# tlemane/kmtricks

Measured on AMD Instinct MI355X. Metric: k-mers merged/s (merge stage, sum over partitions of input records / time), higher is better.
Workload: dtype u64 keys / u32 counts (integer)

## Files before the change

kmtricks_amd/csrc/kmx_api.hip:

```cpp
#include "kmx_host.hpp"

#include <algorithm>
#include <chrono>
#include <cmath>
#include <sys/mman.h>
#include <unordered_map>
#include <mutex>
#include <cstdlib>
#include <cstring>
#include <memory>

using namespace kmx;

static thread_local std::string g_create_err;

void* kmx_ctx::dalloc(size_t bytes)
{
  if (bytes == 0) bytes = 256;
  if (bytes >= (8u << 20)) { size_t p2 = (size_t)1 << 23; while (p2 * 2 <= bytes) p2 *= 2; const size_t q = p2 >> 3; bytes = (bytes + q - 1) / q * q; }
  int best = -1;
  for (size_t i = 0; i < pool.size(); i++)
    if (!pool[i].used && pool[i].bytes >= bytes && pool[i].bytes <= 2 * bytes + (1u << 20) &&
        (best < 0 || pool[i].bytes < pool[best].bytes)) best = (int)i;
  if (best >= 0) { pool[best].used = true; return pool[best].p; }
// ... 388 lines not shown
  size_t o_recs = 0, o_len = 0, o_smin = 0, o_bounds = 0, o_stats = 0, o_ctrl = 0, o_segs = 0;
  u8* d_out = nullptr; size_t out_bytes = 0;
  u16* d_rowrec = nullptr;
  u32 bft_c = 1;
  u8* d_img = nullptr; size_t img_bytes = 0;
  u64 t_rows = 0, t_cols = 0;
  Seg* d_segs = nullptr;
  Seg* d_segs_own = nullptr;
  u64 rows = 0, nsegs = 0;
  bool done = false;
  bool handed_back = false;
  u32 nblk = 0, nb = 0, rt_cols = 0, slots_cap = 0;
  size_t o_skel = 0, o_nskel = 0, o_rbounds = 0;
  u8* d_ov = nullptr;
  size_t o_spdir = 0;
  size_t o_ovx = 0; u32 xcap = 0;
  u64 sparse_rows = 0;
  u8* d_body = nullptr;
  bool body_ready = false;
  hipEvent_t ev_body = nullptr;
  void* d_body_tmp = nullptr;
  u8* d_dense = nullptr; u32 dpitch = 0, dense_cap = 0; size_t o_gbase = 0;
  u8* d_narrow = nullptr; u32 npitch = 0;
  u64 row_keys = 0;
  bool ordered = false;
  std::vector<u32> src;
  int kernel = 0;
};

struct kmx_merge_result {
// ... 94 lines not shown
    const TaskDev* d_subs = reinterpret_cast<const TaskDev*>(R->d_meta + R->o_subtasks);
    const uint2* d_subitems = reinterpret_cast<const uint2*>(R->d_meta + R->o_subitems);
    const ColsDev* d_cols = reinterpret_cast<const ColsDev*>(R->d_meta + R->o_cols);
    const uint2* d_citems = reinterpret_cast<const uint2*>(R->d_meta + R->o_citems);
    static const bool overlap = getenv("KMX_COLS_PREP_OVERLAP") != nullptr;
    hipStream_t ps = overlap ? ctx->aux : ctx->stream;
    if (!R->ev_pre) KMX_HIP(ctx, hipEventCreateWithFlags(&R->ev_pre, hipEventDisableTiming));
    if (overlap && ctx->stream_shared) {
      KMX_HIP(ctx, hipEventRecord(R->ev_pre, ctx->stream));
      KMX_HIP(ctx, hipStreamWaitEvent(ctx->aux, R->ev_pre, 0));
    }
    if (!overlap) KMX_HIP(ctx, hipStreamWaitEvent(ctx->stream, R->ev_up, 0));
    KMX_HIP(ctx, launch_range_bounds(kw, d_subs, nt, R->sub_max_n, R->sub_max_c, ps));
    KMX_HIP(ctx, CO.skel(d_subs, d_subitems, R->n_subitems, ps));
    KMX_HIP(ctx, CO.prep(d_tasks, d_subs, d_cols, nt, ps));
    KMX_HIP(ctx, hipEventRecord(R->ev_pre, ps));
    KMX_HIP(ctx, hipStreamWaitEvent(ctx->stream, R->ev_up, 0));
    KMX_HIP(ctx, launch_range_bounds(kw, d_tasks, nt, R->max_n, R->max_c, ctx->stream));
    KMX_HIP(ctx, hipStreamWaitEvent(ctx->stream, R->ev_pre, 0));
    if (R->ev0) KMX_HIP(ctx, hipEventRecord(R->ev0, ctx->stream));
    const u32 cols_grid_env = getenv("KMX_COLS_GRID") ? (u32)atoi(getenv("KMX_COLS_GRID")) : 0u;
    const u32 sparse_cus_env = getenv("KMX_SPARSE_CUS") ? (u32)atoi(getenv("KMX_SPARSE_CUS")) : 0u;
    KMX_HIP(ctx, CO.merge(mode, (R->cols_ext ? 1 : 0) | (R->cols_resc ? 2 : 0) | (R->cols_ord ? 4 : 0) | (R->cols_narrow ? 8 : 0), d_tasks, d_cols, d_citems, R->n_citems, d_ticket,
                          cols_grid_env ? std::min(cols_grid_env, R->cols_grid) : R->cols_grid, ctx->stream));
    if (R->ev0) { if (!R->ev_mid) KMX_HIP(ctx, hipEventCreate(&R->ev_mid)); KMX_HIP(ctx, hipEventRecord(R->ev_mid, ctx->stream)); }
    KMX_HIP(ctx, CO.sparse(mode | (R->cols_resc ? 2 : 0) | (R->cols_ord ? 4 : 0), d_tasks, d_cols, d_items, R->n_items, nt, d_ticket, sparse_cus_env ? std::min(sparse_cus_env, (u32)ctx->n_cu) : (u32)ctx->n_cu, ctx->stream));
    if (R->share_fix) {
      if ((size_t)R->max_n * 4 > 48 * 1024) KMX_HIP(ctx, hipFuncSetAttribute(reinterpret_cast<const void*>(&k_share_fix), hipFuncAttributeMaxDynamicSharedMemorySize, (int)std::min<size_t>((size_t)R->max_n * 4, 160 * 1024)));
      hipLaunchKernelGGL(k_share_fix, dim3((unsigned)ctx->n_cu * 2u, nt), dim3(256), (size_t)R->max_n * 4, ctx->stream, (const TaskDev*)d_tasks, kw);
      KMX_HIP(ctx, hipGetLastError());
// ... 357 lines not shown
  R->d_meta = (u8*)ctx->dalloc(off);
  R->h_meta = (u8*)ctx->halloc(upload_bytes);
  if (!R->d_meta || !R->h_meta) { ctx->dfree(R->d_meta); ctx->hfree(R->h_meta); return ctx->fail(KMX_E_NOMEM, "meta allocation failed"); }
  auto drop_blocks = [&]() {
    for (auto& G : R->tasks) { ctx->dfree(G.d_out); ctx->dfree(G.d_ov); ctx->dfree(G.d_img); ctx->dfree(G.d_rowrec); ctx->dfree(G.d_dense); ctx->dfree(G.d_narrow); }
    for (auto& G : R->subs) ctx->dfree(G.d_out);
    ctx->dfree(R->d_meta); ctx->hfree(R->h_meta); ctx->dfree(R->d_rem); R->d_rem = nullptr;
  };
  bool narrow_failed = false;
  for (auto& H : R->tasks) {
    H.d_out = (u8*)ctx->dalloc(H.out_bytes);
    if (H.d_out && cols) {
      H.xcap = (u32)std::min<u64>(0x7FFFFF00ULL, CO.ext_entries(H.slots_cap, H.nblk));
      H.o_ovx = align_up((size_t)(CO.scratch_keys(H.slots_cap, H.nblk) * 8 + CO.scratch_counts(H.slots_cap, H.nblk) * 8), 256);
      H.o_spdir = align_up(H.o_ovx + (size_t)H.xcap * (CO.key_words + 1) * 8, 256);
      H.d_ov = (u8*)ctx->dalloc(H.o_spdir + 256 + (size_t)CO.dir_bytes(H.slots_cap));
      if (H.d_ov && hipMemsetAsync(H.d_ov + H.o_spdir, 0, 256 + (size_t)CO.dir_bytes(H.slots_cap), ctx->aux) != hipSuccess) { ctx->dfree(H.d_ov); H.d_ov = nullptr; }
      if (R->cols_ord) {
        const TaskHost& Q = R->subs[&H - R->tasks.data()];
        u64 longest = 0, sum = 0; for (u32 l : Q.len) { longest = std::max<u64>(longest, l); sum += l; }
        u64 cap = (H.rec_min <= 1 ? std::min<u64>(sum, longest * 5 / 2) : longest * 3 / 2) + 4096;
        if (ctx->keys_per_longest > 0.0) cap = std::max<u64>(cap, (u64)(ctx->keys_per_longest * 1.25 * (double)longest) + 4096);
        H.dense_cap = (u32)std::min<u64>(std::min<u64>(cap, H.out_cap_rows), 0xFFFFFF00ULL);
        H.dpitch = (u32)align_up(H.row_bytes - 8 * kw, 8);
        H.d_dense = (u8*)ctx->dalloc((size_t)H.dense_cap * H.dpitch);
        if (R->cols_narrow) {
          H.npitch = (u32)align_up((size_t)H.N, 16) + 16;
          H.d_narrow = (u8*)ctx->dalloc((size_t)H.dense_cap * H.npitch);
          if (!H.d_narrow) narrow_failed = true;
        }
      }
// ... 61 lines not shown
      }
      fill_dev(Q, sd[t]);
      sd[t].item0 = si;
      for (u32 j = 0; j < Q.c; j++) sitems[si++] = make_uint2(t, j);
      ColsDev& C = cd[t];
      C.skel = reinterpret_cast<u64*>(R->d_meta + H.o_skel);
      C.nskel = reinterpret_cast<u32*>(R->d_meta + H.o_nskel);
      C.rbounds = reinterpret_cast<u32*>(R->d_meta + H.o_rbounds);
      C.ovkeys = reinterpret_cast<u64*>(H.d_ov);
      C.ovcnt = reinterpret_cast<u32*>(H.d_ov + CO.scratch_keys(H.slots_cap, H.nblk) * 8);
      C.ovx = reinterpret_cast<u64*>(H.d_ov + H.o_ovx);
      C.xcur = reinterpret_cast<u32*>(H.d_ov + H.o_spdir);
      C.xcap = H.xcap;
      C.spdir = H.d_ov + H.o_spdir + 256;
      C.slots_cap = H.slots_cap; C.nblk = H.nblk; C.nb = H.nb; C.rt = H.rt_cols;
      if (R->cols_ord) {
        const size_t ng = CO.groups(H.slots_cap);
        C.dense = H.d_dense; C.dpitch = H.dpitch; C.dense_cap = H.dense_cap;
        C.dnarrow = H.d_narrow; C.npitch = H.npitch;
        C.gbase = reinterpret_cast<u32*>(R->d_meta + H.o_gbase);
        C.chain = reinterpret_cast<u64*>(H.d_ov + H.o_spdir + 256);
        C.gmap = reinterpret_cast<uint4*>(H.d_ov + H.o_spdir + 256 + ng * 8);
        C.gmax = reinterpret_cast<u32*>(R->d_meta + R->o_ticket) + 2;
        C.ngcap = (u32)ng;
        u32* const tk3 = reinterpret_cast<u32*>(R->h_meta + R->o_ticket) + 3;
        *tk3 = std::max<u32>(*tk3, (u32)ng);
      }
      for (u32 j = 0; j < H.c * H.nblk; j++) citems[ci++] = make_uint2(t, j);
    }
  }
// ... 450 lines not shown
    st[5 * (u64)N + i] = two + twr;
  }
  return KMX_OK;
}

#ifdef KMX_PHASE_PROF
namespace kmx { void rows_phase_prof_dump(); void pivot_phase_prof_dump(); void bft_phase_prof_dump(); }
#endif
extern "C" void kmx_result_free(kmx_merge_result* R)
{
  if (!R) return;
  kmx_ctx* ctx = R->ctx;
  (void)hipSetDevice(ctx->device);
  if (R->ev_done) (void)hipEventSynchronize(R->ev_done);
  else (void)hipStreamSynchronize(ctx->stream);
#ifdef KMX_PHASE_PROF
  const ColsOps& CO = cols_ops((int)R->tasks[0].kw);
  if (R->is_bft) kmx::bft_phase_prof_dump();
  if (!R->is_bf) { if (R->use_cols) { if (CO.phase_prof_dump) CO.phase_prof_dump(); } else if (R->use_pivot) kmx::pivot_phase_prof_dump(); else kmx::rows_phase_prof_dump(); }
#endif
  for (auto& H : R->tasks) {
    if (H.ev_body) { (void)hipEventSynchronize(H.ev_body); (void)hipEventDestroy(H.ev_body); }
    ctx->dfree(H.d_out); ctx->dfree(H.d_segs_own); ctx->dfree(H.d_ov); ctx->dfree(H.d_img); ctx->dfree(H.d_rowrec); ctx->dfree(H.d_body); ctx->dfree(H.d_body_tmp); ctx->dfree(H.d_dense); ctx->dfree(H.d_narrow);
  }
  for (auto& Q : R->subs) ctx->dfree(Q.d_out);
  ctx->dfree(R->d_meta);
  ctx->hfree(R->h_meta);
  ctx->dfree(R->d_in);
  ctx->dfree(R->d_rem);
  if (R->ev_in) (void)hipEventDestroy(R->ev_in);
// ... 548 lines not shown
```

kmtricks_amd/csrc/kmx_dev.hpp:

```cpp
#pragma once
#include <hip/hip_runtime.h>
#include <stdint.h>

namespace kmx {

typedef unsigned long long u64;
typedef uint32_t u32;
typedef uint16_t u16;
typedef uint8_t u8;
typedef __attribute__((address_space(1))) const u32 gu32;

struct Seg {
  u32 range;
  u32 seq;
  u64 row_off;
  u32 nrows;
  u32 pad;
};

struct TaskDev {
  const u8* const* recs;
  const u32* len;
  const u32* soft_min;
  u32* bounds;
// ... 28 lines not shown
  void* spdir;
  u32 slots_cap;
  u32 nblk;
  u32 nb;
  u32 rt;
  u8* dense;
  u32 dpitch;
  u32 dense_cap;
  u8* dnarrow;
  u32 npitch;
  u32* gbase;
  u64* chain;
  uint4* gmap;
  u32* gmax;
  u32 ngcap;
};

#ifndef KMX_CHUNK_BYTES
#define KMX_CHUNK_BYTES 262144
#endif

enum { ERR_ROWS_OVERFLOW = 1, ERR_SEGS_OVERFLOW = 2, ERR_FALLBACK = 4,
       ERR_DIVERGENT = 8,
       ERR_SLICES = 16,
       ERR_DENSE_CAP = 32 };

template <int KW> struct Key { u64 w[KW]; };

template <int KW> __device__ __forceinline__ bool key_less(const Key<KW>& a, const Key<KW>& b) {
#pragma unroll
// ... 67 lines not shown
```

kmtricks_amd/csrc/kmx_host.hpp:

```cpp
#pragma once
#include <hip/hip_runtime.h>
#include <string>
#include <functional>
#include <vector>
#include "kmx_dev.hpp"
#include "skf.hpp"
#include "../../include/kmx.h"

namespace kmx {

int rows_lds_bytes(int kw, u32 n_lists);
int rows_cap(int kw, u32 n_lists);
int rows_wgs_per_cu(int kw);
u32 rows_chunk_rows(u32 row_bytes);
u32 rows_image_bytes(int kw);
hipError_t launch_range_bounds(int kw, const TaskDev* tasks, u32 n_tasks, u32 max_n, u32 max_c, hipStream_t st);
hipError_t launch_merge_rows(int kw, int mode, const TaskDev* tasks, const uint2* items, u32 n_items, u32* ticket,
                             u32 grid_x, u32 max_n, hipStream_t st);
int rows_s_cap(int kw, u32 n_lists);
int rows_s_wgs_per_cu(int kw);
u32 rows_s_image_bytes(int kw);
hipError_t launch_merge_rows_s(int kw, int mode, const TaskDev* tasks, const uint2* items, u32 n_items, u32* ticket, u32 grid_x, u32 max_n, hipStream_t st);
int pivot_lds_bytes(int kw);
u32 pivot_max_lists();
hipError_t launch_merge_pivot(int kw, int mode, const TaskDev* tasks, const uint2* items, u32 n_items, u32* ticket,
                              u32 grid_x, hipStream_t st);
struct ColsOps {
  int (*lds_bytes)();
  u32 (*block_lists)();
  u32 (*wgs_per_cu)();
  u32 (*tile_rows)(u32 nb);
  u64 (*scratch_keys)(u32 slots, u32 nblk);
  u64 (*scratch_counts)(u32 slots, u32 nblk);
  u64 (*ext_entries)(u32 slots, u32 nblk);
  u32 (*skel_cap)();
  hipError_t (*skel)(const TaskDev* subs, const uint2* items, u32 n_items, hipStream_t st);
  hipError_t (*prep)(const TaskDev* tasks, const TaskDev* subs, const ColsDev* cols, u32 n_tasks, hipStream_t st);
  hipError_t (*merge)(int mode, int ext, const TaskDev* tasks, const ColsDev* cols, const uint2* items, u32 n_items, u32* ticket, u32 grid_x, hipStream_t st);
  hipError_t (*sparse)(int mode, const TaskDev* tasks, const ColsDev* cols, const uint2* range_items, u32 n_items, u32 n_tasks, u32* ticket, u32 n_cu, hipStream_t st);
  u64 (*dir_bytes)(u32 slots);
  u32 (*groups)(u32 slots);
  hipError_t (*offsets)(const ColsDev* cols, u32 task, u64* goff, hipStream_t st);
  hipError_t (*gather)(const TaskDev* tasks, const ColsDev* cols, u32 task, u32 n_groups, const u64* goff, u8* body, hipStream_t st);
  hipError_t (*order)(const TaskDev* tasks, const ColsDev* cols, u32 task, u32 n_groups, const u64* goff, u32* order, hipStream_t st);
  void (*dbg_dump)();
  void (*phase_prof_dump)();
  u32 key_words;
};
const ColsOps& cols_ops_k1();
const ColsOps& cols_ops_k2();
inline const ColsOps& cols_ops(int kw) { return kw == 2 ? cols_ops_k2() : cols_ops_k1(); }
int bf_lds_bytes(u32 rt, u32 nb, u32 n_lists);
hipError_t launch_range_bounds_bf(const TaskDev* tasks, u32 n_tasks, u32 max_n, u32 max_c, hipStream_t st);
hipError_t launch_merge_bf(int bfc, const TaskDev* tasks, const uint2* items, u32 n_items, u32* ticket,
                           u32 grid_x, int lds, hipStream_t st);
u32 bft_tile_rows(u32 rec_min, u32 share_min);
u32 bft_block_lists();
u32 bft_max_lists();
u32 bft_round_records(bool wide);
u32 bft_fit_rows(u32 max_n, bool bits);
// ... 182 lines not shown
```

kmtricks_amd/csrc/merge_cols.hip:

```cpp
#include "kmx_host.hpp"
#include <algorithm>
#include <cstdio>
#include <cstring>

#ifndef KMX_CL_KW
#define KMX_CL_KW 1
#endif
#if KMX_CL_KW == 1
#define CLNS cols_k1
#elif KMX_CL_KW == 2
#define CLNS cols_k2
#elif KMX_CL_KW == 3
#define CLNS cols_k3
#else
#define CLNS cols_k4
#endif

namespace kmx { namespace CLNS {

#ifndef KMX_CL_TPB
#define KMX_CL_TPB 1024
#endif
constexpr int CL_TPB = KMX_CL_TPB;
constexpr int CL_WGS = 1024 / CL_TPB;
// ... 3 lines not shown
constexpr int CL_G = KMX_CL_G;
constexpr int KW = KMX_CL_KW;
constexpr int RB = KW * 8 + 4;
constexpr int RD = RB / 4;
constexpr int EW = KW + 1;
constexpr int CL_U = KW == 1 ? 16 : 8;
constexpr int CL_W = CL_G * CL_U;
constexpr int CL_NB = CL_TPB / CL_G;
constexpr int CL_IMG = 61440 / CL_WGS;
constexpr int CL_RT = CL_W * 7 / 8;
constexpr int CL_KPL = (CL_RT + 63) / 64;
constexpr int CL_NT = (CL_KPL == 1 && CL_WGS == 1 && KW == 1) ? 2 : 1;
constexpr int CL_PT = CL_KPL == 1 ? 2048 : 4096;
constexpr int CL_PTSHIFT = CL_PT == 2048 ? 21 : 20;
constexpr int CL_HALVES = CL_KPL;
constexpr int CL_SEEDS = 256;
constexpr int CL_OVW = 128;
constexpr int CL_XS = 3 * CL_OVW;
constexpr int CL_NW = CL_TPB / 64;
constexpr int CK_BITS = 1 << 17;
constexpr int CP_MAXSEG = 2048;

__device__ u32 kmx_cols_dbg[16];

namespace {

typedef u32 u32x3 __attribute__((ext_vector_type(3), aligned(4)));
typedef u32 u32x4 __attribute__((ext_vector_type(4), aligned(4)));
typedef __attribute__((address_space(1))) const u32x3 gu32x3;
typedef __attribute__((address_space(1))) const u32x4 gu32x4;
typedef __attribute__((address_space(1))) u64 gu64w;
// ... 60 lines not shown
  return ((u32)__umul24(x, hf) >> CL_PTSHIFT) & (u32)(CL_PT - 1);
}
__device__ __forceinline__ u32 cl_mult(u32 seed)
{
  if (KW == 2 && seed >= 16u) return 0x80000000u | (seed - 15u);
  if (seed >= 64u) return 0x80000000u | (seed - 63u);
  return ((0x9E3779u + seed * 0x5A6B2u) & 0xFFFFFFu) | ((13u + (seed * 7u) % 19u) << 24);
}
__device__ __forceinline__ u32 cl_mix(CKey key)
{
  const u64 k = ck_fold(key);
  u32 x = (u32)k ^ ((u32)(k >> 32) * 0x9E3779B1u);
  x *= 0x85EBCA6Bu; x ^= x >> 15; x *= 0x2C1B3C6Du; x ^= x >> 13;
  return x;
}
__device__ __forceinline__ u32 cl_build(ClEnt* tab, const CKey (&key)[CL_KPL], const bool (&have)[CL_KPL], u32 lane, u32 (&slot)[CL_KPL])
{
  for (u32 s = 0; s < (u32)CL_SEEDS; s++) {
    const u32 mult = cl_mult(s);
    u32 h[CL_KPL], old[CL_KPL];
    bool clash = false;
#pragma unroll
    for (int x = 0; x < CL_KPL; x++) {
      h[x] = cl_thash(key[x], mult);
      old[x] = have[x] ? atomicCAS(&tab[h[x]].idx, 0u, lane + 64u * x + 1) : 0u;
      clash |= old[x] != 0;
    }
    if (__ballot(clash) == 0) {
#pragma unroll
      for (int x = 0; x < CL_KPL; x++) { if (have[x]) ent_set(tab[h[x]], key[x]); slot[x] = h[x]; }
      return mult;
    }
#pragma unroll
    for (int x = 0; x < CL_KPL; x++) if (have[x] && old[x] == 0) atomicExch(&tab[h[x]].idx, 0u);
  }
  return 0;
}

}

#ifndef KMX_SK_TPB
#define KMX_SK_TPB 256
#endif
constexpr int SK_TPB = KMX_SK_TPB;
constexpr int SK_CAP = 2048;

__global__ __launch_bounds__(SK_TPB)
void k_cols_skel(const TaskDev* __restrict__ subs, const uint2* __restrict__ items, u32 n_items)
{
  __shared__ CKey ks[SK_CAP];
  __shared__ u32 wsum[SK_TPB / 64];
// ... 156 lines not shown
      u32 g = 0;
      for (u32 j = 0; j < T.c; j++) { C.gbase[j] = g; const u32 n = C.rbounds[j + 1] - C.rbounds[j]; g += max(1u, (n + C.rt - 1) / C.rt) * (u32)CL_HALVES; }
      C.gbase[T.c] = g; s_ng = g;
      atomicMax(C.gmax, g);
    }
    __syncthreads();
    const u32 ng = s_ng;
    for (u32 g = tid; g < ng; g += CP_TPB) {
      u32 lo = 0, hi = T.c;
      while (hi - lo > 1) { const u32 mid = (lo + hi) >> 1; if (C.gbase[mid] <= g) lo = mid; else hi = mid; }
      C.gmap[g] = make_uint4(lo + 1, g - C.gbase[lo], C.rbounds[lo], C.rbounds[lo + 1]);
    }
  }
}

__device__ const u32 kmx_cols_sentinel[8] = {~0u, ~0u, KW == 1 ? 0u : ~0u, KW == 1 ? 0u : ~0u, 0u, 0u, 0u, 0u};

#ifdef KMX_PHASE_PROF
__device__ u64 kmx_cols_prof[8];
__device__ u64 kmx_sparse_prof[8];
#ifndef KMX_PROF_TID
#define KMX_PROF_TID 512
#endif
#endif

constexpr u64 CL_NONSOLID = 1ULL << 63;
template <int MODE, bool EXT, bool RESC, bool ORD, bool NAR>
__global__ __launch_bounds__(CL_TPB, CL_WGS)
void k_merge_cols(const TaskDev* __restrict__ tasks, const ColsDev* __restrict__ cols, const uint2* __restrict__ items,
                  u32 n_items, u32* ticket)
{
// ... 54 lines not shown
    const u32 end = on ? T.bounds[(u64)(range + 1) * N + li] : 0u;
    const u32 smin = T.soft_min[li];
    gu32* const base = (gu32*)(uintptr_t)T.recs[li];
    gu32* const sentinel = (gu32*)(uintptr_t)kmx_cols_sentinel;
    CRec rec[CL_U];
#pragma unroll
    for (int u = 0; u < CL_U; u++) {
      const u32 ix = cur + ((r + CL_G * u - cur) & (CL_W - 1));
      rec[u] = cl_none();
      if (ix < end) rec[u] = cl_load(base + (u64)ix * RD);
    }
    u64 tsum = 0; u32 tn = 0;
    u64 rsum = 0; u32 rn = 0;
    const bool rescue = RESC && cl_uni(T.share_min) != 0;
    CKey skn[CL_KPL];
    u32 myslot[CL_KPL];
    bool failed = false;
#pragma unroll
    for (int x = 0; x < CL_KPL; x++) { skn[x] = ck_inf(); myslot[x] = 0; }
    if (tid < 64) {
      bool have[CL_KPL];
#pragma unroll
      for (int x = 0; x < CL_KPL; x++) {
        const u32 j = (u32)tid + 64u * x;
        have[x] = j < rt && s_lo + j < s_hi;
        if (have[x]) {
          skn[x] = skel[s_lo + j];
          if (blk == 0 && !ord) ck_store(reinterpret_cast<u32*>(T.out + (u64)(s_lo + j) * row_bytes), skn[x]);
        }
      }
      const u32 mult = cl_build(ptab, skn, have, (u32)tid, myslot);
      if (tid == 0) { sh[4] = mult; if (mult == 0) { failed = true; atomicAdd(&kmx_cols_dbg[0], 1u); } }
    }
    CKey khi_n = ntiles > 1 ? skel[s_lo + rt] : ck_inf();
    CKey kmid_n = (CL_HALVES > 1 && s_lo + 56 < s_hi) ? skel[s_lo + 56] : ck_inf();
    u32 rnd = 0;
    cl_barrier();
    CLPH(0);

    for (u32 q = 0; q < ntiles; q++) {
      const u32 s0 = s_lo + q * rt;
      const u32 rte = min(rt, s_hi - s0);
      const bool last = cl_uni(q + 1 == ntiles ? 1u : 0u) != 0;
      const CKey khi = ck_uni(khi_n);
      const CKey kmid = ck_uni(kmid_n);
      if (!last) {
        if (tid < 64) {
#pragma unroll
          for (int x = 0; x < CL_KPL; x++) { const u32 j = (u32)tid + 64u * x; skn[x] = ck_inf(); if (j < rt && s0 + rt + j < s_hi) skn[x] = skel[s0 + rt + j]; }
        }
        khi_n = q + 2 < ntiles ? skel[s0 + 2 * rt] : ck_inf();
        kmid_n = (CL_HALVES > 1 && s0 + rt + 56 < s_hi) ? skel[s0 + rt + 56] : ck_inf();
      }
      const ClEnt* const tab = ptab + (q % CL_NT) * CL_PT;
      const u32 mult = cl_uni(sh[4 + (q % CL_NT)]);
      gu64w* const ovk0 = (gu64w*)(uintptr_t)(C.ovkeys + (((((u64)(slot0 + q) * CL_HALVES) * nblk + blk) * CL_NW + wave) * CL_OVW) * EW);
      gu64w* const ovk1 = ovk0 + (u64)nblk * CL_NW * CL_OVW * EW;
      const u64 li_hi = (u64)li << 32;
      u32 wov = 0, wov1 = 0;
      u32 xb0 = 0, xb1 = 0;
      auto extend = [&](u32& xb) {
        u32 b = 0;
        if (lane == 0) b = atomicAdd(C.xcur, (u32)CL_XS);
        b = cl_uni(b);
        xb = (b + (u32)CL_XS <= C.xcap) ? b + 1u : 0xFFFFFFFFu;
      };
      gu64w* const ovx = (gu64w*)(uintptr_t)C.ovx;

      for (;;) {
        if (tid == 0) sh[1 + (rnd == 2 ? 0 : rnd + 1)] = 0;
// ... 107 lines not shown
        const u32 more = cl_uni(sh[1 + rnd]);
        rnd = rnd == 2 ? 0 : rnd + 1;
        if (!more) break;
      }
      if (lane == 0) {
        const u64 s0i = (((u64)(slot0 + q) * CL_HALVES) * nblk + blk) * CL_NW + wave, s1i = (((u64)(slot0 + q) * CL_HALVES + 1) * nblk + blk) * CL_NW + wave;
        reinterpret_cast<uint2*>(C.ovcnt)[s0i] = make_uint2(wov, xb0 == 0xFFFFFFFFu ? 0u : xb0);
        if (CL_HALVES > 1) reinterpret_cast<uint2*>(C.ovcnt)[s1i] = make_uint2(wov1, xb1 == 0xFFFFFFFFu ? 0u : xb1);
        const bool over0 = wov > (u32)CL_OVW && (xb0 - 1u >= 0xFFFFFFFEu || wov > (u32)(CL_OVW + CL_XS));
        const bool over1 = wov1 > (u32)CL_OVW && (xb1 - 1u >= 0xFFFFFFFEu || wov1 > (u32)(CL_OVW + CL_XS));
        if (over0 || over1) {
          if (lane == 0) atomicOr(&T.ctrl[2], (u64)ERR_SLICES); failed = true; atomicAdd(&kmx_cols_dbg[1], 1u); atomicMax(&kmx_cols_dbg[5], max(wov, wov1)); if (last) atomicAdd(&kmx_cols_dbg[6], 1u); if (q == 0) atomicAdd(&kmx_cols_dbg[7], 1u); }
      }

      if (wave == 0) {
        ClEnt* const old = ptab + (q % CL_NT) * CL_PT;
#pragma unroll
        for (int x = 0; x < CL_KPL; x++) if ((u32)lane + 64u * x < rte) old[myslot[x]].idx = 0;
        if (!last) {
          const u32 sn = s0 + rt;
          bool have[CL_KPL];
#pragma unroll
          for (int x = 0; x < CL_KPL; x++) {
            const u32 j = (u32)lane + 64u * x;
            have[x] = j < rt && sn + j < s_hi;
            if (have[x] && blk == 0 && !ord) ck_store(reinterpret_cast<u32*>(T.out + (u64)(sn + j) * row_bytes), skn[x]);
          }
          const u32 m2 = cl_build(ptab + ((q + 1) % CL_NT) * CL_PT, skn, have, (u32)lane, myslot);
          if (lane == 0) { sh[4 + ((q + 1) % CL_NT)] = m2; if (m2 == 0) { failed = true; atomicAdd(&kmx_cols_dbg[0], 1u); } }
        }
      } else {
        if (NAR) {
          const u32 lr = (u32)lane >> 3, lc = (u32)lane & 7u, nch = (nbl + 15u) >> 4;
          for (u32 j = (wave - 1) * 8u + lr; j < rte; j += (CL_NW - 1) * 8u) {
            u8* const nrow = nar + (u64)(s0 + j) * npitch;
            if (lc < nch) {
              uint4* const src = reinterpret_cast<uint4*>(img8 + j * nbs + 16u * lc);
              const uint4 v = *src; *src = make_uint4(0, 0, 0, 0);
              *reinterpret_cast<uint4*>(nrow + col0 + 16u * lc) = v;
            }
            if (lc == 0) { const u8 f = rowbig[j]; rowbig[j] = 0; nrow[npitch - 16u + blk] = f; }
          }
        } else
        if (MODE == 0) {
// ... 55 lines not shown
      }
      if (RESC) {
        u32 rlo = (u32)rsum, rhi = (u32)(rsum >> 32);
        u64 rs = rsum;
#pragma unroll
        for (int off = 1; off < CL_G; off <<= 1) {
          const u32 olo = __shfl_xor(rlo, off), ohi = __shfl_xor(rhi, off);
          rs += (u64)olo | ((u64)ohi << 32);
          rlo = (u32)rs; rhi = (u32)(rs >> 32);
          rn += __shfl_xor(rn, off);
        }
        if (on && r == 0 && rn) { atomicAdd(&T.stats[1 * (u64)N + li], (u64)rn); atomicAdd(&T.stats[5 * (u64)N + li], rs); }
      }
    }
    if (failed) atomicOr(&T.ctrl[2], (u64)ERR_FALLBACK);
    __syncthreads();
  }
}

#ifndef KMX_CK_TPB0
#define KMX_CK_TPB0 256
#endif
#ifndef KMX_CK_TPB1
#define KMX_CK_TPB1 512
#endif
#ifndef KMX_CK_Z
#define KMX_CK_Z 16
#endif
#ifndef KMX_CK_OCC1
#define KMX_CK_OCC1 4
// ... 887 lines not shown
      }
    } else if ((row_bytes & 3u) == 0) for (u32 t = lane; t < row_bytes / 4; t += 64) reinterpret_cast<u32*>(d)[t] = reinterpret_cast<const u32*>(s)[t];
    else for (u32 t = lane; t < row_bytes; t += 64) d[t] = s[t];
  }
}

void cols_dbg_dump()
{
  u32 h[16];
  if (hipMemcpyFromSymbol(h, HIP_SYMBOL(kmx_cols_dbg), sizeof(h)) != hipSuccess) return;
  if (h[9]) fprintf(stderr, "[kmx merge] k_cols_sparse: the group count of the batch was beyond every task's room (%u workgroups stopped at the room)\n", h[9]);
  if (h[8]) fprintf(stderr, "[kmx merge] k_cols_sparse: %u look-backs given up (last: group %u, %u entries still unpublished in front of it)\n", h[8], h[10], h[11]);
  fprintf(stderr, "[kmx merge] k_merge_cols hand-back reasons: no collision-free row table %u, slice overflow %u (wave-tiles; largest %u, in a range's last tile %u, first tile %u), kept key outside the row keys %u, check table full %u, lists too divergent %u (tasks)\n", h[0], h[1], h[5], h[6], h[7], h[2], h[3], h[4]);
  memset(h, 0, sizeof(h)); (void)hipMemcpyToSymbol(HIP_SYMBOL(kmx_cols_dbg), h, sizeof(h));
}
#ifdef KMX_PHASE_PROF
void cols_phase_prof_dump()
{
  u64 h[8];
  if (hipMemcpyFromSymbol(h, HIP_SYMBOL(kmx_cols_prof), sizeof(h)) != hipSuccess) return;
  u64 tot = 0; for (int i = 0; i < 8; i++) tot += h[i];
  static const char* nm[8] = {"item setup", "window wait", "scan", "bar(scan)", "tile out", "bar(out)", "-", "-"};
  for (int i = 0; i < 6; i++) fprintf(stderr, "[cols] %-12s %6.2f%%  %llu\n", nm[i], tot ? 100.0 * h[i] / tot : 0.0, h[i]);
  memset(h, 0, sizeof(h));
  (void)hipMemcpyToSymbol(HIP_SYMBOL(kmx_cols_prof), h, sizeof(h));
  if (hipMemcpyFromSymbol(h, HIP_SYMBOL(kmx_sparse_prof), sizeof(h)) != hipSuccess) return;
  tot = 0; for (int i = 0; i < 8; i++) tot += h[i];
  static const char* sn[8] = {"group entries", "zero maps", "mark twice | sample + place", "candidates | rank", "sort", "runs + claim", "rows", "gather (rec-min 1)"};
  for (int i = 0; i < 8; i++) fprintf(stderr, "[sparse] %-14s %6.2f%%  %llu\n", sn[i], tot ? 100.0 * h[i] / tot : 0.0, h[i]);
  memset(h, 0, sizeof(h));
// ... 9 lines not shown
u64 cols_scratch_keys(u32 slots, u32 nblk) { return (u64)slots * CL_HALVES * nblk * CL_NW * CL_OVW * EW; }
u64 cols_scratch_counts(u32 slots, u32 nblk) { return (u64)slots * CL_HALVES * nblk * CL_NW; }
u64 cols_ext_entries(u32 slots, u32 nblk) { return std::max<u64>(64 * 1024, (u64)slots * CL_HALVES * nblk * CL_NW * CL_OVW / 16); }

u32 cols_skel_cap() { return SK_CAP; }
hipError_t launch_cols_skel(const TaskDev* subs, const uint2* items, u32 n_items, hipStream_t st)
{
  hipLaunchKernelGGL(k_cols_skel, dim3(n_items), dim3(SK_TPB), 0, st, subs, items, n_items);
  return hipGetLastError();
}
hipError_t launch_cols_prep(const TaskDev* tasks, const TaskDev* subs, const ColsDev* cols, u32 n_tasks, hipStream_t st)
{
  hipLaunchKernelGGL(k_cols_prep, dim3(n_tasks), dim3(CP_TPB), 0, st, tasks, subs, cols);
  return hipGetLastError();
}
template <int MODE, bool EXT, bool RESC, bool ORD, bool NAR>
static hipError_t launch_merge_cols_as(const TaskDev* tasks, const ColsDev* cols, const uint2* items, u32 n_items, u32* ticket, u32 grid_x, hipStream_t st)
{
  const int lds = cols_lds_bytes();
  hipError_t e = hipFuncSetAttribute(reinterpret_cast<const void*>(&k_merge_cols<MODE, EXT, RESC, ORD, NAR>), hipFuncAttributeMaxDynamicSharedMemorySize, lds);
  if (e != hipSuccess) return e;
  hipLaunchKernelGGL((k_merge_cols<MODE, EXT, RESC, ORD, NAR>), dim3(grid_x), dim3(CL_TPB), lds, st, tasks, cols, items, n_items, ticket);
  return hipGetLastError();
}
hipError_t launch_merge_cols(int mode, int ext, const TaskDev* tasks, const ColsDev* cols, const uint2* items, u32 n_items, u32* ticket, u32 grid_x, hipStream_t st)
{
  const bool x = ext & 1, r = (ext & 2) != 0, o = (ext & 4) != 0, n = (ext & 8) != 0 && o && mode == 0;
#define KMX_CL_L3(M, X, R) (o ? launch_merge_cols_as<M, X, R, true, false>(tasks, cols, items, n_items, ticket, grid_x, st) : launch_merge_cols_as<M, X, R, false, false>(tasks, cols, items, n_items, ticket, grid_x, st))
#define KMX_CL_LAUNCH(M) (r ? (x ? KMX_CL_L3(M, true, true) : KMX_CL_L3(M, false, true)) : (x ? KMX_CL_L3(M, true, false) : KMX_CL_L3(M, false, false)))
  if (n) return r ? (x ? launch_merge_cols_as<0, true, true, true, true>(tasks, cols, items, n_items, ticket, grid_x, st) : launch_merge_cols_as<0, false, true, true, true>(tasks, cols, items, n_items, ticket, grid_x, st))
// ... 40 lines not shown
  hipLaunchKernelGGL(k_cols_offsets, dim3(1), dim3(1024), 0, st, cols, task, goff);
  return hipGetLastError();
}
hipError_t launch_cols_gather(const TaskDev* tasks, const ColsDev* cols, u32 task, u32 n_groups, const u64* goff, u8* body, hipStream_t st)
{
  hipLaunchKernelGGL(k_cols_gather<true>, dim3(n_groups), dim3(GA_TPB), 0, st, tasks, cols, task, goff, body);
  return hipGetLastError();
}
hipError_t launch_cols_order(const TaskDev* tasks, const ColsDev* cols, u32 task, u32 n_groups, const u64* goff, u32* order, hipStream_t st)
{
  hipLaunchKernelGGL(k_cols_gather<false>, dim3(n_groups), dim3(GA_TPB), 0, st, tasks, cols, task, goff, reinterpret_cast<u8*>(order));
  return hipGetLastError();
}

static const ColsOps g_ops = {cols_lds_bytes, cols_block_lists, cols_wgs_per_cu, cols_tile_rows, cols_scratch_keys, cols_scratch_counts, cols_ext_entries, cols_skel_cap,
                              launch_cols_skel, launch_cols_prep, launch_merge_cols, launch_cols_sparse, cols_dir_bytes, cols_groups, launch_cols_offsets,
                              launch_cols_gather, launch_cols_order, cols_dbg_dump,
#ifdef KMX_PHASE_PROF
                              cols_phase_prof_dump,
#else
                              nullptr,
#endif
                              (u32)KMX_CL_KW};
}
#if KMX_CL_KW == 1
const ColsOps& cols_ops_k1() { return cols_k1::g_ops; }
#elif KMX_CL_KW == 2
const ColsOps& cols_ops_k2() { return cols_k2::g_ops; }
#elif KMX_CL_KW == 3
const ColsOps& cols_ops_k3() { return cols_k3::g_ops; }
#else
const ColsOps& cols_ops_k4() { return cols_k4::g_ops; }
// ... 3 lines not shown
```

Measured before the change: 127.8 billion.

## Precompute collision-free hash seeds per tile in a separate prep kernel

Adds a k_cols_seeds kernel on the prep stream that searches each tile's hash multiplier with an LDS bitmap instead of CAS on the row table, storing seeds in a new per-slot tseed array. The merge kernel then just reads the seed and fills the table directly, dropping the CAS/retry build and per-tile slot clearing in favor of a full table clear at the end. Seed search moves off the critical merge path and can overlap with other prep work, but it adds a kernel launch and extra memory, and raises the try limit to 1024.

```diff
diff --git a/kmtricks_amd/csrc/kmx_api.hip b/kmtricks_amd/csrc/kmx_api.hip
--- a/kmtricks_amd/csrc/kmx_api.hip
+++ b/kmtricks_amd/csrc/kmx_api.hip
@@ -426,6 +426,7 @@
   size_t o_skel = 0, o_nskel = 0, o_rbounds = 0;
   u8* d_ov = nullptr;
   size_t o_spdir = 0;
+  size_t o_tseed = 0;
   size_t o_ovx = 0; u32 xcap = 0;
   u64 sparse_rows = 0;
   u8* d_body = nullptr;
@@ -550,6 +551,12 @@
     KMX_HIP(ctx, launch_range_bounds(kw, d_subs, nt, R->sub_max_n, R->sub_max_c, ps));
     KMX_HIP(ctx, CO.skel(d_subs, d_subitems, R->n_subitems, ps));
     KMX_HIP(ctx, CO.prep(d_tasks, d_subs, d_cols, nt, ps));
+    {
+      u32 max_slots = 0;
+      for (auto& H : R->tasks) max_slots = std::max(max_slots, H.slots_cap);
+      const char* const tenv = getenv("KMX_COLS_SEED_TRIES");
+      KMX_HIP(ctx, CO.seeds(d_tasks, d_cols, nt, max_slots, tenv && atoi(tenv) > 0 ? (u32)atoi(tenv) : 0u, getenv("KMX_TRACE") != nullptr, ps));
+    }
     KMX_HIP(ctx, hipEventRecord(R->ev_pre, ps));
     KMX_HIP(ctx, hipStreamWaitEvent(ctx->stream, R->ev_up, 0));
     KMX_HIP(ctx, launch_range_bounds(kw, d_tasks, nt, R->max_n, R->max_c, ctx->stream));
@@ -937,7 +944,8 @@
       H.xcap = (u32)std::min<u64>(0x7FFFFF00ULL, CO.ext_entries(H.slots_cap, H.nblk));
       H.o_ovx = align_up((size_t)(CO.scratch_keys(H.slots_cap, H.nblk) * 8 + CO.scratch_counts(H.slots_cap, H.nblk) * 8), 256);
       H.o_spdir = align_up(H.o_ovx + (size_t)H.xcap * (CO.key_words + 1) * 8, 256);
-      H.d_ov = (u8*)ctx->dalloc(H.o_spdir + 256 + (size_t)CO.dir_bytes(H.slots_cap));
+      H.o_tseed = align_up(H.o_spdir + 256 + (size_t)CO.dir_bytes(H.slots_cap), 256);
+      H.d_ov = (u8*)ctx->dalloc(H.o_tseed + (size_t)H.slots_cap * 4);
       if (H.d_ov && hipMemsetAsync(H.d_ov + H.o_spdir, 0, 256 + (size_t)CO.dir_bytes(H.slots_cap), ctx->aux) != hipSuccess) { ctx->dfree(H.d_ov); H.d_ov = nullptr; }
       if (R->cols_ord) {
         const TaskHost& Q = R->subs[&H - R->tasks.data()];
@@ -1029,6 +1037,7 @@
       C.xcap = H.xcap;
       C.spdir = H.d_ov + H.o_spdir + 256;
       C.slots_cap = H.slots_cap; C.nblk = H.nblk; C.nb = H.nb; C.rt = H.rt_cols;
+      C.tseed = reinterpret_cast<u32*>(H.d_ov + H.o_tseed);
       if (R->cols_ord) {
         const size_t ng = CO.groups(H.slots_cap);
         C.dense = H.d_dense; C.dpitch = H.dpitch; C.dense_cap = H.dense_cap;
@@ -1509,6 +1518,7 @@
   (void)hipSetDevice(ctx->device);
   if (R->ev_done) (void)hipEventSynchronize(R->ev_done);
   else (void)hipStreamSynchronize(ctx->stream);
+  if (R->use_cols && getenv("KMX_TRACE")) cols_ops((int)R->tasks[0].kw).seeds_dump();
 #ifdef KMX_PHASE_PROF
   const ColsOps& CO = cols_ops((int)R->tasks[0].kw);
   if (R->is_bft) kmx::bft_phase_prof_dump();
diff --git a/kmtricks_amd/csrc/kmx_dev.hpp b/kmtricks_amd/csrc/kmx_dev.hpp
--- a/kmtricks_amd/csrc/kmx_dev.hpp
+++ b/kmtricks_amd/csrc/kmx_dev.hpp
@@ -66,6 +66,7 @@
   uint4* gmap;
   u32* gmax;
   u32 ngcap;
+  u32* tseed;
 };
 
 #ifndef KMX_CHUNK_BYTES
diff --git a/kmtricks_amd/csrc/kmx_host.hpp b/kmtricks_amd/csrc/kmx_host.hpp
--- a/kmtricks_amd/csrc/kmx_host.hpp
+++ b/kmtricks_amd/csrc/kmx_host.hpp
@@ -36,6 +36,7 @@
   u32 (*skel_cap)();
   hipError_t (*skel)(const TaskDev* subs, const uint2* items, u32 n_items, hipStream_t st);
   hipError_t (*prep)(const TaskDev* tasks, const TaskDev* subs, const ColsDev* cols, u32 n_tasks, hipStream_t st);
+  hipError_t (*seeds)(const TaskDev* tasks, const ColsDev* cols, u32 n_tasks, u32 max_slots, u32 max_tries, bool trace, hipStream_t st);
   hipError_t (*merge)(int mode, int ext, const TaskDev* tasks, const ColsDev* cols, const uint2* items, u32 n_items, u32* ticket, u32 grid_x, hipStream_t st);
   hipError_t (*sparse)(int mode, const TaskDev* tasks, const ColsDev* cols, const uint2* range_items, u32 n_items, u32 n_tasks, u32* ticket, u32 n_cu, hipStream_t st);
   u64 (*dir_bytes)(u32 slots);
@@ -44,6 +45,7 @@
   hipError_t (*gather)(const TaskDev* tasks, const ColsDev* cols, u32 task, u32 n_groups, const u64* goff, u8* body, hipStream_t st);
   hipError_t (*order)(const TaskDev* tasks, const ColsDev* cols, u32 task, u32 n_groups, const u64* goff, u32* order, hipStream_t st);
   void (*dbg_dump)();
+  void (*seeds_dump)();
   void (*phase_prof_dump)();
   u32 key_words;
 };
diff --git a/kmtricks_amd/csrc/merge_cols.hip b/kmtricks_amd/csrc/merge_cols.hip
--- a/kmtricks_amd/csrc/merge_cols.hip
+++ b/kmtricks_amd/csrc/merge_cols.hip
@@ -41,7 +41,6 @@
 constexpr int CL_PT = CL_KPL == 1 ? 2048 : 4096;
 constexpr int CL_PTSHIFT = CL_PT == 2048 ? 21 : 20;
 constexpr int CL_HALVES = CL_KPL;
-constexpr int CL_SEEDS = 256;
 constexpr int CL_OVW = 128;
 constexpr int CL_XS = 3 * CL_OVW;
 constexpr int CL_NW = CL_TPB / 64;
@@ -132,27 +131,33 @@
   x *= 0x85EBCA6Bu; x ^= x >> 15; x *= 0x2C1B3C6Du; x ^= x >> 13;
   return x;
 }
-__device__ __forceinline__ u32 cl_build(ClEnt* tab, const CKey (&key)[CL_KPL], const bool (&have)[CL_KPL], u32 lane, u32 (&slot)[CL_KPL])
-{
-  for (u32 s = 0; s < (u32)CL_SEEDS; s++) {
+__device__ __forceinline__ u32 cl_find(u32* bm, const CKey (&key)[CL_KPL], const bool (&have)[CL_KPL], u32 lane, u32 max_tries, u32& tries)
+{
+  for (u32 s = 0; s < max_tries; s++) {
     const u32 mult = cl_mult(s);
-    u32 h[CL_KPL], old[CL_KPL];
+    for (u32 w = lane; w < (u32)CL_PT / 32u; w += 64u) bm[w] = 0;
+    __builtin_amdgcn_wave_barrier();
     bool clash = false;
 #pragma unroll
     for (int x = 0; x < CL_KPL; x++) {
-      h[x] = cl_thash(key[x], mult);
-      old[x] = have[x] ? atomicCAS(&tab[h[x]].idx, 0u, lane + 64u * x + 1) : 0u;
-      clash |= old[x] != 0;
-    }
-    if (__ballot(clash) == 0) {
-#pragma unroll
-      for (int x = 0; x < CL_KPL; x++) { if (have[x]) ent_set(tab[h[x]], key[x]); slot[x] = h[x]; }
-      return mult;
-    }
-#pragma unroll
-    for (int x = 0; x < CL_KPL; x++) if (have[x] && old[x] == 0) atomicExch(&tab[h[x]].idx, 0u);
-  }
+      const u32 h = cl_thash(key[x], mult);
+      if (have[x]) clash |= ((atomicOr(&bm[h >> 5], 1u << (h & 31u)) >> (h & 31u)) & 1u) != 0;
+    }
+    __builtin_amdgcn_wave_barrier();
+    if (__ballot(clash) == 0) { tries = s + 1; return mult; }
+  }
+  tries = max_tries;
   return 0;
+}
+__device__ __forceinline__ void cl_fill(ClEnt* tab, const CKey (&key)[CL_KPL], const bool (&have)[CL_KPL], u32 lane, u32 mult)
+{
+#pragma unroll
+  for (int x = 0; x < CL_KPL; x++) {
+    if (have[x]) {
+      ClEnt e; memset(&e, 0, sizeof(e)); ent_set(e, key[x]); e.idx = lane + 64u * x + 1;
+      tab[cl_thash(key[x], mult)] = e;
+    }
+  }
 }
 
 }
@@ -339,7 +344,52 @@
   }
 }
 
-__device__ const u32 kmx_cols_sentinel[8] = {~0u, ~0u, KW == 1 ? 0u : ~0u, KW == 1 ? 0u : ~0u, 0u, 0u, 0u, 0u};
+constexpr int CS_TPB = 256;
+constexpr u32 CS_TRIES = 1024;
+__device__ u32 kmx_cols_tries[12];
+__global__ __launch_bounds__(CS_TPB)
+void k_cols_seeds(const TaskDev* __restrict__ tasks, const ColsDev* __restrict__ cols, u32 max_tries, u32 trace)
+{
+  __shared__ u32 bm[CS_TPB / 64][CL_PT / 32];
+  __shared__ u32 s_fail;
+  const TaskDev& T = tasks[blockIdx.y];
+  const ColsDev& C = cols[blockIdx.y];
+  const u32 tid = threadIdx.x, lane = tid & 63u, wave = tid >> 6;
+  if (tid == 0) s_fail = 0;
+  if (__syncthreads_or((__hip_atomic_load(&T.ctrl[2], __ATOMIC_RELAXED, __HIP_MEMORY_SCOPE_AGENT) & (u64)(ERR_FALLBACK | ERR_ROWS_OVERFLOW)) != 0)) return;
+  const u32 slot = blockIdx.x * (u32)(CS_TPB / 64) + wave, c = T.c, rt = C.rt;
+  if (slot < C.slots_cap && slot <= C.rbounds[c] / rt + c) {
+    u32 lo = 0, hi = c;
+    while (hi - lo > 1) { const u32 mid = (lo + hi) >> 1; if (C.rbounds[mid] / rt + mid <= slot) lo = mid; else hi = mid; }
+    const u32 s_lo = C.rbounds[lo], s_hi = C.rbounds[lo + 1];
+    const u32 q = slot - (s_lo / rt + lo), ntiles = max(1u, (s_hi - s_lo + rt - 1) / rt);
+    if (q < ntiles) {
+      const u32 s0 = s_lo + q * rt;
+      CKey key[CL_KPL]; bool have[CL_KPL];
+#pragma unroll
+      for (int x = 0; x < CL_KPL; x++) {
+        const u32 j = lane + 64u * x;
+        have[x] = j < rt && s0 + j < s_hi;
+        key[x] = have[x] ? reinterpret_cast<const CKey*>(C.skel)[s0 + j] : ck_inf();
+      }
+      u32 tries = 0;
+      const u32 mult = cl_find(bm[wave], key, have, lane, max_tries, tries);
+      if (lane == 0) {
+        C.tseed[slot] = mult;
+        if (mult == 0) { s_fail = 1; atomicAdd(&kmx_cols_dbg[0], 1u); }
+        if (trace) {
+          u32 b = 0; while (b < 8u && (1u << b) < tries) b++;
+          atomicAdd(&kmx_cols_tries[mult == 0 ? 11u : s0 >= s_hi ? 9u : b], 1u);
+          atomicMax(&kmx_cols_tries[10], tries);
+        }
+      }
+    }
+  }
+  __syncthreads();
+  if (tid == 0 && s_fail) atomicOr(&T.ctrl[2], (u64)ERR_FALLBACK);
+}
+
+__device__ const u32 kmx_cols_sentinel[8] ={~0u, ~0u, KW == 1 ? 0u : ~0u, KW == 1 ? 0u : ~0u, 0u, 0u, 0u, 0u};
 
 #ifdef KMX_PHASE_PROF
 __device__ u64 kmx_cols_prof[8];
@@ -424,10 +474,9 @@
     u64 rsum = 0; u32 rn = 0;
     const bool rescue = RESC && cl_uni(T.share_min) != 0;
     CKey skn[CL_KPL];
-    u32 myslot[CL_KPL];
     bool failed = false;
 #pragma unroll
-    for (int x = 0; x < CL_KPL; x++) { skn[x] = ck_inf(); myslot[x] = 0; }
+    for (int x = 0; x < CL_KPL; x++) skn[x] = ck_inf();
     if (tid < 64) {
       bool have[CL_KPL];
 #pragma unroll
@@ -439,8 +488,9 @@
           if (blk == 0 && !ord) ck_store(reinterpret_cast<u32*>(T.out + (u64)(s_lo + j) * row_bytes), skn[x]);
         }
       }
-      const u32 mult = cl_build(ptab, skn, have, (u32)tid, myslot);
-      if (tid == 0) { sh[4] = mult; if (mult == 0) { failed = true; atomicAdd(&kmx_cols_dbg[0], 1u); } }
+      const u32 m0 = cl_uni(C.tseed[slot0]);
+      cl_fill(ptab, skn, have, (u32)tid, m0);
+      if (tid == 0) sh[5] = m0;
     }
     CKey khi_n = ntiles > 1 ? skel[s_lo + rt] : ck_inf();
     CKey kmid_n = (CL_HALVES > 1 && s_lo + 56 < s_hi) ? skel[s_lo + 56] : ck_inf();
@@ -454,7 +504,9 @@
       const bool last = cl_uni(q + 1 == ntiles ? 1u : 0u) != 0;
       const CKey khi = ck_uni(khi_n);
       const CKey kmid = ck_uni(kmid_n);
+      const u32 mult = cl_uni(sh[5]);
       if (!last) {
+        if (tid == 0) sh[4] = C.tseed[slot0 + q + 1];
         if (tid < 64) {
 #pragma unroll
           for (int x = 0; x < CL_KPL; x++) { const u32 j = (u32)tid + 64u * x; skn[x] = ck_inf(); if (j < rt && s0 + rt + j < s_hi) skn[x] = skel[s0 + rt + j]; }
@@ -463,7 +515,6 @@
         kmid_n = (CL_HALVES > 1 && s0 + rt + 56 < s_hi) ? skel[s0 + rt + 56] : ck_inf();
       }
       const ClEnt* const tab = ptab + (q % CL_NT) * CL_PT;
-      const u32 mult = cl_uni(sh[4 + (q % CL_NT)]);
       gu64w* const ovk0 = (gu64w*)(uintptr_t)(C.ovkeys + (((((u64)(slot0 + q) * CL_HALVES) * nblk + blk) * CL_NW + wave) * CL_OVW) * EW);
       gu64w* const ovk1 = ovk0 + (u64)nblk * CL_NW * CL_OVW * EW;
       const u64 li_hi = (u64)li << 32;
@@ -601,9 +652,6 @@
       }
 
       if (wave == 0) {
-        ClEnt* const old = ptab + (q % CL_NT) * CL_PT;
-#pragma unroll
-        for (int x = 0; x < CL_KPL; x++) if ((u32)lane + 64u * x < rte) old[myslot[x]].idx = 0;
         if (!last) {
           const u32 sn = s0 + rt;
           bool have[CL_KPL];
@@ -613,8 +661,9 @@
             have[x] = j < rt && sn + j < s_hi;
             if (have[x] && blk == 0 && !ord) ck_store(reinterpret_cast<u32*>(T.out + (u64)(sn + j) * row_bytes), skn[x]);
           }
-          const u32 m2 = cl_build(ptab + ((q + 1) % CL_NT) * CL_PT, skn, have, (u32)lane, myslot);
-          if (lane == 0) { sh[4 + ((q + 1) % CL_NT)] = m2; if (m2 == 0) { failed = true; atomicAdd(&kmx_cols_dbg[0], 1u); } }
+          const u32 m2 = cl_uni(sh[4]);
+          cl_fill(ptab + ((q + 1) % CL_NT) * CL_PT, skn, have, (u32)lane, m2);
+          if (lane == 0) sh[5] = m2;
         }
       } else {
         if (NAR) {
@@ -700,6 +749,8 @@
       }
     }
     if (failed) atomicOr(&T.ctrl[2], (u64)ERR_FALLBACK);
+    int t0 = tid; asm volatile("" : "+v"(t0));
+    for (int t = t0; t < CL_NT * CL_PT; t += CL_TPB) ptab[t].idx = 0;
     __syncthreads();
   }
 }
@@ -1617,6 +1668,16 @@
   fprintf(stderr, "[kmx merge] k_merge_cols hand-back reasons: no collision-free row table %u, slice overflow %u (wave-tiles; largest %u, in a range's last tile %u, first tile %u), kept key outside the row keys %u, check table full %u, lists too divergent %u (tasks)\n", h[0], h[1], h[5], h[6], h[7], h[2], h[3], h[4]);
   memset(h, 0, sizeof(h)); (void)hipMemcpyToSymbol(HIP_SYMBOL(kmx_cols_dbg), h, sizeof(h));
 }
+void cols_seeds_dump()
+{
+  u32 h[12];
+  if (hipMemcpyFromSymbol(h, HIP_SYMBOL(kmx_cols_tries), sizeof(h)) != hipSuccess) return;
+  u64 n = 0; for (int i = 0; i < 10; i++) n += h[i];
+  if (n + h[11] == 0) return;
+  fprintf(stderr, "[kmx merge] k_cols_seeds: hash words tried per tile: 1: %u, 2: %u, 3-4: %u, 5-8: %u, 9-16: %u, 17-32: %u, 33-64: %u, 65-128: %u, more: %u; tiles without row keys %u, most tries %u, none found %u\n",
+          h[0], h[1], h[2], h[3], h[4], h[5], h[6], h[7], h[8], h[9], h[10], h[11]);
+  memset(h, 0, sizeof(h)); (void)hipMemcpyToSymbol(HIP_SYMBOL(kmx_cols_tries), h, sizeof(h));
+}
 #ifdef KMX_PHASE_PROF
 void cols_phase_prof_dump()
 {
@@ -1656,6 +1717,12 @@
   hipLaunchKernelGGL(k_cols_prep, dim3(n_tasks), dim3(CP_TPB), 0, st, tasks, subs, cols);
   return hipGetLastError();
 }
+hipError_t launch_cols_seeds(const TaskDev* tasks, const ColsDev* cols, u32 n_tasks, u32 max_slots, u32 max_tries, bool trace, hipStream_t st)
+{
+  const u32 per = (u32)(CS_TPB / 64);
+  hipLaunchKernelGGL(k_cols_seeds, dim3((max_slots + per - 1) / per, n_tasks), dim3(CS_TPB), 0, st, tasks, cols, max_tries ? max_tries : CS_TRIES, trace ? 1u : 0u);
+  return hipGetLastError();
+}
 template <int MODE, bool EXT, bool RESC, bool ORD, bool NAR>
 static hipError_t launch_merge_cols_as(const TaskDev* tasks, const ColsDev* cols, const uint2* items, u32 n_items, u32* ticket, u32 grid_x, hipStream_t st)
 {
@@ -1726,8 +1793,8 @@
 }
 
 static const ColsOps g_ops = {cols_lds_bytes, cols_block_lists, cols_wgs_per_cu, cols_tile_rows, cols_scratch_keys, cols_scratch_counts, cols_ext_entries, cols_skel_cap,
-                              launch_cols_skel, launch_cols_prep, launch_merge_cols, launch_cols_sparse, cols_dir_bytes, cols_groups, launch_cols_offsets,
-                              launch_cols_gather, launch_cols_order, cols_dbg_dump,
+                              launch_cols_skel, launch_cols_prep, launch_cols_seeds, launch_merge_cols, launch_cols_sparse, cols_dir_bytes, cols_groups, launch_cols_offsets,
+                              launch_cols_gather, launch_cols_order, cols_dbg_dump, cols_seeds_dump,
 #ifdef KMX_PHASE_PROF
                               cols_phase_prof_dump,
 #else
```

Result: faster. 132.1 billion, median of 6 (+3.4%).
